# IrisRainbowNeko/HCP-Diffusion

Hardware: AMD Instinct MI355X
Metric: training images/sec (whole node), SD1.5 LoRA 512px bs=4/GPU (higher is better)
Workload: dtype bf16; 1 GPU; SD1.5 UNet LoRA rank=8 bf16, bs=4/GPU, 512x512 (64x64 latents), 77-token context, random-init weights, cached latents, grad-ckpt off; global_batch=4, parallelism=dp1, rccl_ranks=1, comm=none, hip_graph=True, gradient_checkpointing=False

## Files before the change

### hcp_diffusion_amd/csrc/attention.hip

```cpp
#include "attn_dma.h"

namespace {
using namespace hcp_attn;

HCP_KERNEL(256) attn_dkv_convert_kernel(AttnParams p, int B, int C) {
    const int cv = C / 4;
    const long total = (long)B * p.Nk * cv;
    const size_t slab = (size_t)B * p.Nk * C;
    for (long i = (long)blockIdx.x * blockDim.x + threadIdx.x; i < total; i += (long)gridDim.x * blockDim.x) {
        const int c = (int)(i % cv) * 4; long r = i / cv; const int n = (int)(r % p.Nk); const int b = (int)(r / p.Nk);
        const size_t e = ((size_t)b * p.Nk + n) * C + c;
        hcp_f32x4 k4 = *(const hcp_f32x4*)(p.dk32 + e);
        hcp_f32x4 v4 = *(const hcp_f32x4*)(p.dv32 + e);
        for (int s = 1; s < p.qsplit; ++s) {
            const hcp_f32x4 ks = *(const hcp_f32x4*)(p.dk32 + s * slab + e); k4 += ks;
            const hcp_f32x4 vs = *(const hcp_f32x4*)(p.dv32 + s * slab + e); v4 += vs;
        }
        hcp_bf16x4 wk, wv;
#pragma unroll
        for (int q = 0; q < 4; ++q) { wk[q] = (short)hcp_f2bf(k4[q]); wv[q] = (short)hcp_f2bf(v4[q]); }
        *(hcp_bf16x4*)(p.dK + (size_t)b * p.k_bs + (size_t)n * p.k_rs + c) = wk;
        *(hcp_bf16x4*)(p.dV + (size_t)b * p.v_bs + (size_t)n * p.v_rs + c) = wv;
    }
}

constexpr int kMinQTilesPerSplit = 16, kSplitTargetWgs = 256;
HCP_TUNABLE(int, g_attn_cfg, -1);

constexpr int VAR_FWD = VAR_PRODUCT | VAR_LSUM;
constexpr int VAR_PRE_BASE = VAR_XCD | VAR_ONES | VAR_PRE;
constexpr int VAR_FWD_PRE = VAR_PRE_BASE | VAR_LSUM;
template <int D, int QT, int NW>
int launch_fwd(AttnParams& p, int B, hipStream_t stream) {
    const int n = hcp_cdiv(p.Nq, 16 * QT * NW) * p.H * B;
    if (p.kbias || p.causal) HCP_LAUNCH((attn2_fwd_kernel<D, QT, true, VAR_PRODUCT, NW>), dim3(n), dim3(64 * NW), fwd_smem<D>(), stream, p);
    else if (p.pre) HCP_LAUNCH((attn2_fwd_kernel<D, QT, false, VAR_FWD_PRE, NW>), dim3(n), dim3(64 * NW), fwd_smem<D>(), stream, p);
    else HCP_LAUNCH((attn2_fwd_kernel<D, QT, false, VAR_FWD, NW>), dim3(n), dim3(64 * NW), fwd_smem<D>(), stream, p);
    HCP_LAUNCH_CHECK("attn_fwd");
}
template <int D, int QT>
int launch_dq(AttnParams& p, int B, hipStream_t stream) {
    const int n = hcp_cdiv(p.Nq, 64 * QT) * p.H * B;
    if (p.kbias || p.causal) HCP_LAUNCH((attn2_bwd_dq_kernel<D, QT, true, VAR_PRODUCT>), dim3(n), dim3(256), fwd_smem<D>(), stream, p);
    else if (p.pre) HCP_LAUNCH((attn2_bwd_dq_kernel<D, QT, false, VAR_PRE_BASE>), dim3(n), dim3(256), fwd_smem<D>(), stream, p);
    else HCP_LAUNCH((attn2_bwd_dq_kernel<D, QT, false, VAR_PRODUCT>), dim3(n), dim3(256), fwd_smem<D>(), stream, p);
    HCP_LAUNCH_CHECK("attn_bwd_dq");
}
template <int D, int KT>
void plan_dkv(AttnParams& p, int B, float* ws, size_t ws_bytes) {
    const int nkv = hcp_cdiv(p.Nk, 64 * KT);
    const int nqt = hcp_cdiv(p.Nq, KVT);
    int qsplit = 1;
    const long base = (long)nkv * p.H * B;
    const size_t need1 = (size_t)2 * B * p.Nk * p.H * D * sizeof(float);
    if (base < 256 && nqt >= 8 && ws && ws_bytes >= 2 * need1) {
        const bool ovr = g_attn_cfg >= 0 && (g_attn_cfg >> 8);
        const int min_tiles = ovr ? ((g_attn_cfg >> 8) & 255) : kMinQTilesPerSplit;
        const int target = ovr ? 256 * ((g_attn_cfg >> 16) & 15) : kSplitTargetWgs;
        qsplit = (int)((target + base - 1) / base);
        if (qsplit > nqt / min_tiles) qsplit = nqt / min_tiles;
        if ((size_t)qsplit > ws_bytes / need1) qsplit = (int)(ws_bytes / need1);
        if (qsplit < 2) qsplit = 1;
    }
    p.qsplit = qsplit;
    if (qsplit > 1) { p.dk32 = ws; p.dv32 = ws + (size_t)qsplit * B * p.Nk * p.H * D; }
}
template <int D, int KT>
int launch_dkv(AttnParams& p, int B, hipStream_t stream) {
    const int nkv = hcp_cdiv(p.Nk, 64 * KT);
    const int qsplit = p.qsplit;
    const int n = nkv * qsplit * p.H * B;
    if (p.kbias || p.causal) HCP_LAUNCH((attn2_bwd_dkv_kernel<D, KT, true, VAR_PRODUCT>), dim3(n), dim3(256), dkv_smem<D>(), stream, p);
    else if (p.pre) HCP_LAUNCH((attn2_bwd_dkv_kernel<D, KT, false, VAR_PRE_BASE>), dim3(n), dim3(256), dkv_smem<D>(), stream, p);
    else HCP_LAUNCH((attn2_bwd_dkv_kernel<D, KT, false, VAR_PRODUCT>), dim3(n), dim3(256), dkv_smem<D>(), stream, p);
    if (qsplit > 1) {
        long tot = (long)B * p.Nk * (p.H * D / 4);
        int g = (int)((tot + 255) / 256); if (g > 2048) g = 2048;
        HCP_LAUNCH(attn_dkv_convert_kernel, dim3(g), dim3(256), 0, stream, p, B, p.H * D);
    }
    HCP_LAUNCH_CHECK("attn_bwd_dkv");
}

template <int D> constexpr bool kWide = D <= 64;

template <int D>
int run_fwd(AttnParams& p, int B, hipStream_t stream) {
    const long bh = (long)B * p.H;
    bool wide = kWide<D> && bh * hcp_cdiv(p.Nq, 128) >= 512;
    bool w8 = (D == 40 || D == 80) && bh * hcp_cdiv(p.Nq, D == 40 ? 256 : 128) >= 256;
    if (g_attn_cfg >= 0 && !(g_attn_cfg & 16)) { wide = kWide<D> && (g_attn_cfg & 1); w8 = (D == 40 || D == 80) && (g_attn_cfg & 8); }
    if constexpr (D == 40) {
        if (w8) return wide ? launch_fwd<D, 2, 8>(p, B, stream) : launch_fwd<D, 1, 8>(p, B, stream);
        return wide ? launch_fwd<D, 2, 4>(p, B, stream) : launch_fwd<D, 1, 4>(p, B, stream);
    } else if constexpr (D == 80) {
        return w8 ? launch_fwd<D, 1, 8>(p, B, stream) : launch_fwd<D, 1, 4>(p, B, stream);
    } else if constexpr (kWide<D>) {
        return wide ? launch_fwd<D, 2, 4>(p, B, stream) : launch_fwd<D, 1, 4>(p, B, stream);
    } else {
        return launch_fwd<D, 1, 4>(p, B, stream);
    }
}
template <int D>
int run_bwd(AttnParams& p, int B, float* ws, size_t ws_bytes, hipStream_t stream) {
    bool wq = kWide<D> && (long)B * p.H * hcp_cdiv(p.Nq, 128) >= 512, wk = kWide<D> && (long)B * p.H * hcp_cdiv(p.Nk, 128) >= 512;
    if (g_attn_cfg >= 0 && !(g_attn_cfg & 16)) { wq = kWide<D> && (g_attn_cfg & 2); wk = kWide<D> && (g_attn_cfg & 4); }
    if constexpr (kWide<D>) { if (wk) plan_dkv<D, 2>(p, B, ws, ws_bytes); else plan_dkv<D, 1>(p, B, ws, ws_bytes); }
    else plan_dkv<D, 1>(p, B, ws, ws_bytes);
    int e;
    if constexpr (kWide<D>) { e = wq ? launch_dq<D, 2>(p, B, stream) : launch_dq<D, 1>(p, B, stream); }
    else e = launch_dq<D, 1>(p, B, stream);
    if (e) return e;
    if constexpr (kWide<D>) { return wk ? launch_dkv<D, 2>(p, B, stream) : launch_dkv<D, 1>(p, B, stream); }
    return launch_dkv<D, 1>(p, B, stream);
}

int attn_check(const AttnParams& p, int B, int D) {
    HCP_REQUIRE(B > 0 && p.H > 0 && p.Nq > 0 && p.Nk > 0, "attention: empty problem");
    HCP_REQUIRE(D == 40 || D == 64 || D == 80 || D == 160, "attention: head_dim %d unsupported (40/64/80/160)", D);
    HCP_REQUIRE(p.q_rs % 8 == 0 && p.k_rs % 8 == 0 && p.v_rs % 8 == 0 && p.o_rs % 8 == 0, "attention: row strides must be multiples of 8");
    HCP_REQUIRE(p.q_bs % 8 == 0 && p.k_bs % 8 == 0 && p.v_bs % 8 == 0 && p.o_bs % 8 == 0, "attention: batch strides must be multiples of 8");
    return 0;
}

}

#if defined(HCP_TOOLS)
HCP_API int hcp_debug_set_attention_config(int cfg) { g_attn_cfg = cfg; return 0; }
#endif

HCP_API int hcp_attention_fwd(const void* Q, const void* K, const void* V, void* O, float* lse, int B, int H, int Nq, int Nk,
                              int D, long q_bs, int q_rs, long k_bs, int k_rs, long v_bs, int v_rs, long o_bs, int o_rs,
                              float scale, const float* key_bias, long key_bias_bs, int causal, hipStream_t stream) {
    AttnParams p = {};
    p.kbias = key_bias; p.kb_bs = key_bias_bs; p.causal = causal & 1; p.pre = (causal >> 1) & 1; p.B = B;
    p.Q = (const hcp_bf16*)Q; p.K = (const hcp_bf16*)K; p.V = (const hcp_bf16*)V; p.Out = (hcp_bf16*)O; p.lse = lse;
    p.q_bs = q_bs; p.q_rs = q_rs; p.k_bs = k_bs; p.k_rs = k_rs; p.v_bs = v_bs; p.v_rs = v_rs; p.o_bs = o_bs; p.o_rs = o_rs;
    p.H = H; p.Nq = Nq; p.Nk = Nk; p.scale = scale; p.qsplit = 1;
    HCP_REQUIRE(Q && K && V && O && lse, "hcp_attention_fwd: null pointer");
    HCP_REQUIRE(!(causal & 1) || Nq == Nk, "hcp_attention_fwd: causal masking is defined for self-attention (Nq == Nk)");
    HCP_REQUIRE(!(causal & ~3), "hcp_attention_fwd: unknown flag bits (1 = causal, 2 = Q pre-scaled)");
    HCP_REQUIRE(!p.pre || !(key_bias || p.causal), "hcp_attention_fwd: pre-scaled Q is provided for the unmasked kernels only");
    if (int e = attn_check(p, B, D)) return e;
    switch (D) {
        case 40: return run_fwd<40>(p, B, stream);
        case 64: return run_fwd<64>(p, B, stream);
        case 80: return run_fwd<80>(p, B, stream);
        default: return run_fwd<160>(p, B, stream);
    }
}

HCP_API int hcp_attention_bwd(const void* Q, const void* K, const void* V, const void* O, const void* dO, const float* lse,
                              float* delta, void* dQ, void* dK, void* dV, int B, int H, int Nq, int Nk, int D, long q_bs,
                              int q_rs, long k_bs, int k_rs, long v_bs, int v_rs, long o_bs, int o_rs, float scale,
                              const float* key_bias, long key_bias_bs, int causal, void* workspace, size_t workspace_bytes,
                              hipStream_t stream) {
    AttnParams p = {};
    p.kbias = key_bias; p.kb_bs = key_bias_bs; p.causal = causal & 1; p.pre = (causal >> 1) & 1; p.B = B;
    p.Q = (const hcp_bf16*)Q; p.K = (const hcp_bf16*)K; p.V = (const hcp_bf16*)V; p.O = (const hcp_bf16*)O;
    p.dO = (const hcp_bf16*)dO; p.lse = (float*)lse; p.delta = delta;
    p.dQ = (hcp_bf16*)dQ; p.dK = (hcp_bf16*)dK; p.dV = (hcp_bf16*)dV;
    p.q_bs = q_bs; p.q_rs = q_rs; p.k_bs = k_bs; p.k_rs = k_rs; p.v_bs = v_bs; p.v_rs = v_rs; p.o_bs = o_bs; p.o_rs = o_rs;
    p.H = H; p.Nq = Nq; p.Nk = Nk; p.scale = scale; p.qsplit = 1;
    HCP_REQUIRE(Q && K && V && O && dO && lse && delta && dQ && dK && dV, "hcp_attention_bwd: null pointer");
    HCP_REQUIRE(!(causal & 1) || Nq == Nk, "hcp_attention_bwd: causal masking is defined for self-attention (Nq == Nk)");
    HCP_REQUIRE(!(causal & ~3), "hcp_attention_bwd: unknown flag bits (1 = causal, 2 = Q pre-scaled)");
    HCP_REQUIRE(!p.pre || !(key_bias || p.causal), "hcp_attention_bwd: pre-scaled Q is provided for the unmasked kernels only");
    if (int e = attn_check(p, B, D)) return e;
    float* ws = (float*)workspace; const size_t wb = workspace ? workspace_bytes : 0;
    switch (D) {
        case 40: return run_bwd<40>(p, B, ws, wb, stream);
        case 64: return run_bwd<64>(p, B, ws, wb, stream);
        case 80: return run_bwd<80>(p, B, ws, wb, stream);
        default: return run_bwd<160>(p, B, ws, wb, stream);
    }
}
```

Baseline: 211.4 images/sec.

## Add fused short-key attention backward kernel for cross-attention

Adds a specialised backward kernel for attention with few keys (up to 128, or 80 for head_dim 160), as in SD cross-attention with 77 text tokens. Each block keeps all of K and V resident in LDS and loops over query tiles, computing dQ, dK and dV in a single pass instead of separate dQ and dKV kernels. The query dimension is split across blocks to fill the CUs, and the fp32 dK/dV partials are reduced in the existing convert kernel. The cost is large LDS use per block and a partial-sum workspace, and the path falls back to the old kernels when the workspace is too small.

```diff
diff --git a/hcp_diffusion_amd/csrc/attention.hip b/hcp_diffusion_amd/csrc/attention.hip
--- a/hcp_diffusion_amd/csrc/attention.hip
+++ b/hcp_diffusion_amd/csrc/attention.hip
@@ -1,4 +1,5 @@
 #include "attn_dma.h"
+#include "attn_short_key.h"
 
 namespace {
 using namespace hcp_attn;
@@ -81,6 +82,48 @@
     HCP_LAUNCH_CHECK("attn_bwd_dkv");
 }
 
+constexpr int kSkCUs = 256, kSkMinTiles = 1;
+template <int D, int NKB>
+bool plan_sk(AttnParams& p, int B, float* ws, size_t ws_bytes) {
+    if (p.causal || p.Nk > sk_max_keys<D>()) return false;
+    int forced = 0;
+    if (g_attn_cfg >= 0) {
+        if (!(g_attn_cfg & 32)) return false;
+        forced = (g_attn_cfg >> 20) & 255;
+    }
+    const long bh = (long)B * p.H;
+    const int nqt = hcp_cdiv(p.Nq, KVT);
+    int s = forced;
+    if (!s) {
+        s = (int)(kSkCUs * SkGeom<D, NKB>::WAVES / bh);
+        if (s > nqt / kSkMinTiles) s = nqt / kSkMinTiles;
+        if (s < 1) s = 1;
+    }
+    if (s > nqt) s = nqt;
+    s = hcp_cdiv(nqt, hcp_cdiv(nqt, s));
+    if (s > 1) {
+        const size_t one = (size_t)B * p.Nk * p.H * D;
+        if (!ws || ws_bytes / (2 * one * sizeof(float)) < (size_t)s) return false;
+        p.dk32 = ws; p.dv32 = ws + (size_t)s * one;
+    }
+    p.qsplit = s;
+    return true;
+}
+template <int D, int NKB>
+int launch_sk(AttnParams& p, int B, hipStream_t stream) {
+    constexpr size_t smem = SkGeom<D, NKB>::SMEM;
+    const int n = p.qsplit * p.H * B;
+    if (p.kbias) HCP_LAUNCH((attn_sk_bwd_kernel<D, NKB, true, VAR_PRODUCT>), dim3(n), dim3(256), smem, stream, p);
+    else if (p.pre) HCP_LAUNCH((attn_sk_bwd_kernel<D, NKB, false, VAR_PRE_BASE>), dim3(n), dim3(256), smem, stream, p);
+    else HCP_LAUNCH((attn_sk_bwd_kernel<D, NKB, false, VAR_PRODUCT>), dim3(n), dim3(256), smem, stream, p);
+    if (p.qsplit > 1) {
+        long tot = (long)B * p.Nk * (p.H * D / 4);
+        int g = (int)((tot + 255) / 256); if (g > 2048) g = 2048;
+        HCP_LAUNCH(attn_dkv_convert_kernel, dim3(g), dim3(256), 0, stream, p, B, p.H * D);
+    }
+    HCP_LAUNCH_CHECK("attn_bwd_short_key");
+}
+
 template <int D> constexpr bool kWide = D <= 64;
 
 template <int D>
@@ -102,6 +145,10 @@
 }
 template <int D>
 int run_bwd(AttnParams& p, int B, float* ws, size_t ws_bytes, hipStream_t stream) {
+    if constexpr (sk_max_keys<D>() > 80) {
+        if (p.Nk > 80 && plan_sk<D, 8>(p, B, ws, ws_bytes)) return launch_sk<D, 8>(p, B, stream);
+    }
+    if (p.Nk <= 80 && plan_sk<D, 5>(p, B, ws, ws_bytes)) return launch_sk<D, 5>(p, B, stream);
     bool wq = kWide<D> && (long)B * p.H * hcp_cdiv(p.Nq, 128) >= 512, wk = kWide<D> && (long)B * p.H * hcp_cdiv(p.Nk, 128) >= 512;
     if (g_attn_cfg >= 0 && !(g_attn_cfg & 16)) { wq = kWide<D> && (g_attn_cfg & 2); wk = kWide<D> && (g_attn_cfg & 4); }
     if constexpr (kWide<D>) { if (wk) plan_dkv<D, 2>(p, B, ws, ws_bytes); else plan_dkv<D, 1>(p, B, ws, ws_bytes); }
diff --git a/hcp_diffusion_amd/csrc/attn_short_key.h b/hcp_diffusion_amd/csrc/attn_short_key.h
--- /dev/null
+++ b/hcp_diffusion_amd/csrc/attn_short_key.h
@@ -0,0 +1,231 @@
+#pragma once
+#include "attn_dma.h"
+
+namespace hcp_attn {
+
+template <int D, int NKB> struct SkGeom {
+    using G = Geom<D>;
+    static constexpr int NKBE = (NKB + 1) & ~1;
+    static constexpr int NCH = NKBE / 2;
+    static constexpr int NKP = 16 * NKBE;
+    static constexpr int RSP = NKP + 8;
+    static constexpr int NT = NKB * G::NDV;
+    static constexpr int TPW = (NT + 3) / 4;
+    static constexpr size_t KV_BYTES = (size_t)2 * NKP * G::RS * 2;
+    static constexpr size_t QG_BYTES = (size_t)2 * G::IMG * 2;
+    static constexpr size_t PS_BYTES = (size_t)2 * KVT * RSP * 2;
+    static constexpr size_t BIAS_BYTES = (size_t)NKP * 4;
+    static constexpr size_t LDS_CU = 160 * 1024;
+    static constexpr int NBUF = KV_BYTES + 2 * QG_BYTES + PS_BYTES + BIAS_BYTES <= LDS_CU ? 2 : 1;
+    static constexpr size_t SMEM = KV_BYTES + NBUF * QG_BYTES + PS_BYTES + BIAS_BYTES;
+    static constexpr int WAVES = LDS_CU / SMEM >= 2 ? 2 : 1;
+};
+template <int D> constexpr int sk_max_keys() { return D == 160 ? 80 : 128; }
+
+template <int D, int NKB, bool KB, int VAR>
+HCP_WAVES_PER_SIMD((SkGeom<D, NKB>::WAVES)) HCP_KERNEL(256) attn_sk_bwd_kernel(AttnParams p) {
+    using G = Geom<D>;
+    using SG = SkGeom<D, NKB>;
+    constexpr bool PRE = (VAR & VAR_PRE) != 0;
+    constexpr bool RAW = (VAR & VAR_RAW) != 0 && !PRE;
+    static_assert(PRE || RAW, "short-key backward: raw-unit or pre-scaled scores");
+    HCP_DYN_SMEM(smem);
+    hcp_bf16* sK = (hcp_bf16*)smem;
+    hcp_bf16* sV = sK + SG::NKP * G::RS;
+    hcp_bf16* sQG = sV + SG::NKP * G::RS;
+    hcp_bf16* sP = sQG + SG::NBUF * 2 * G::IMG;
+    hcp_bf16* sS = sP + KVT * SG::RSP;
+    float* sB = (float*)(sS + KVT * SG::RSP);
+    const int tid = threadIdx.x, lane = tid & 63, wave = hcp_uniform(tid >> 6);
+    const int fr = lane & 15, fg = lane >> 4;
+    const int S = p.qsplit;
+    int item = blockIdx.x;
+    if (VAR & VAR_XCD) item = xcd_work_item(item, gridDim.x);
+    const int bh = item / S, qs = item - bh * S, h = bh % p.H, b = bh / p.H;
+    const int nqt = (p.Nq + KVT - 1) / KVT;
+    const int per = (nqt + S - 1) / S;
+    const int it0 = qs * per, it1 = it0 + per < nqt ? it0 + per : nqt;
+    const hcp_bf16* Qb = p.Q + (size_t)b * p.q_bs + h * D;
+    const hcp_bf16* Kb = p.K + (size_t)b * p.k_bs + h * D;
+    const hcp_bf16* Vb = p.V + (size_t)b * p.v_bs + h * D;
+    const hcp_bf16* dOb = p.dO + (size_t)b * p.o_bs + h * D;
+    const hcp_bf16* Ob = p.O + (size_t)b * p.o_bs + h * D;
+    const float* lse_b = p.lse + ((size_t)b * p.H + h) * p.Nq;
+    const float cs = RAW ? p.scale * LOG2E : 1.0f;
+
+    for (int i = tid * 8; i < SG::NBUF * 2 * G::IMG; i += 256 * 8) *(hcp_bf16x8*)(sQG + i) = hcp_zero8();
+    for (int i = tid; i < SG::NKP * G::RG; i += 256) {
+        const int row = i / G::RG, g = i - row * G::RG;
+        const bool ok = row < p.Nk && g < G::REALG;
+        *(hcp_bf16x8*)(sK + row * G::RS + g * 8) = ok ? *(const hcp_bf16x8*)(Kb + (size_t)row * p.k_rs + g * 8) : hcp_zero8();
+        *(hcp_bf16x8*)(sV + row * G::RS + g * 8) = ok ? *(const hcp_bf16x8*)(Vb + (size_t)row * p.v_rs + g * 8) : hcp_zero8();
+    }
+    if (KB)
+        for (int i = tid; i < SG::NKP; i += 256)
+            sB[i] = (i < p.Nk && p.kbias) ? p.kbias[(size_t)b * p.kb_bs + i] * (RAW ? 1.0f / p.scale : LOG2E) : 0.f;
+    TileDma<D> dma;
+    dma.init(wave, lane, p.q_rs, p.o_rs);
+    auto nvalid_q = [&](int q0) { const int n = p.Nq - q0; return n < KVT ? n : KVT; };
+    auto fetch = [&](int it, hcp_bf16* dst) {
+        dma.issue(Qb + (size_t)it * KVT * p.q_rs, p.q_rs, dOb + (size_t)it * KVT * p.o_rs, p.o_rs, nvalid_q(it * KVT), dst, wave);
+    };
+    const int qrow = wave * 16 + fr;
+    hcp_bf16x8 of[G::NQK];
+    float lv = 0.f;
+#pragma unroll
+    for (int s = 0; s < G::NQK; ++s) of[s] = hcp_zero8();
+    auto load_o = [&](int it) {
+        const int row = it * KVT + qrow;
+#pragma unroll
+        for (int s = 0; s < G::NQK; ++s) {
+            const int dc = s * 32 + fg * 8;
+            of[s] = (row < p.Nq && dc < D) ? *(const hcp_bf16x8*)(Ob + (size_t)row * p.o_rs + dc) : hcp_zero8();
+        }
+        lv = row < p.Nq ? lse_b[row] : 0.f;
+    };
+    HCP_SYNC();
+    if (it0 < it1) { load_o(it0); fetch(it0, sQG); }
+    hcp_dma_wait_all();
+    HCP_SYNC();
+
+    hcp_f32x4 dk[SG::TPW], dv[SG::TPW];
+#pragma unroll
+    for (int j = 0; j < SG::TPW; ++j) { hcp_f32x4 z = {0.f, 0.f, 0.f, 0.f}; dk[j] = z; dv[j] = z; }
+    const int kfull = fr * G::RS + fg * 8;
+    const int ktail = fr * G::RS + ((G::NFULL * 32 + fg * 8) < D ? G::NFULL * 32 + fg * 8 : D);
+    const int tfrag = (4 * fg + (fr >> 2)) * G::RS + 4 * (fr & 3);
+    const int pfrag = (4 * fg + (fr >> 2)) * SG::RSP + 4 * (fr & 3);
+    hcp_bf16x4 dqw[G::NDV];
+    int dq_row = p.Nq;
+    auto flush_dq = [&]() {
+        if (dq_row < p.Nq) {
+            hcp_bf16* orow = p.dQ + (size_t)b * p.q_bs + (size_t)dq_row * p.q_rs + h * D;
+#pragma unroll
+            for (int d = 0; d < G::NDV; ++d)
+                if (d * 16 + 4 * fg < D) *(hcp_bf16x4*)(orow + d * 16 + 4 * fg) = dqw[d];
+        }
+        dq_row = p.Nq;
+    };
+    for (int it = it0; it < it1; ++it) {
+        const int q0 = it * KVT;
+        const hcp_bf16* sQ = sQG + (SG::NBUF == 2 ? ((it - it0) & 1) : 0) * 2 * G::IMG;
+        const hcp_bf16* sG = sQ + G::IMG;
+        float dpart = 0.f;
+#pragma unroll
+        for (int s = 0; s < G::NQK; ++s) {
+            const hcp_bf16x8 g = *(const hcp_bf16x8*)(sG + wave * 16 * G::RS + (s < G::NFULL ? kfull + s * 32 : ktail));
+#pragma unroll
+            for (int e = 0; e < 8; ++e) dpart += hcp_bf2f((unsigned short)of[s][e]) * hcp_bf2f((unsigned short)g[e]);
+        }
+        dpart += hcp_shfl_xor(dpart, 16); dpart += hcp_shfl_xor(dpart, 32);
+        const float l2 = q0 + qrow < p.Nq ? lv * LOG2E / cs : 0.f;
+        const hcp_f32x4 nl4 = {-l2, -l2, -l2, -l2}, nd4 = {-dpart, -dpart, -dpart, -dpart};
+        flush_dq();
+        if (it + 1 < it1) {
+            load_o(it + 1);
+            if (SG::NBUF == 2) fetch(it + 1, sQG + (((it + 1 - it0) & 1) * 2 * G::IMG));
+        }
+        hcp_f32x4 sc[SG::NKBE], dp[SG::NKBE];
+#pragma unroll
+        for (int s = 0; s < G::NQK; ++s) {
+            const int off = s < G::NFULL ? kfull + s * 32 : ktail;
+            const hcp_bf16x8 qa = *(const hcp_bf16x8*)(sQ + wave * 16 * G::RS + off);
+            const hcp_bf16x8 ga = *(const hcp_bf16x8*)(sG + wave * 16 * G::RS + off);
+#pragma unroll
+            for (int kb = 0; kb < NKB; ++kb) {
+                const hcp_bf16x8 kf = *(const hcp_bf16x8*)(sK + kb * 16 * G::RS + off);
+                const hcp_bf16x8 vf = *(const hcp_bf16x8*)(sV + kb * 16 * G::RS + off);
+                hcp_f32x4 init = nl4;
+                if (s == 0) {
+#pragma unroll
+                    for (int r = 0; r < 4; ++r) if (kb * 16 + 4 * fg + r >= p.Nk) init[r] = -INFINITY;
+                }
+                sc[kb] = hcp_mfma16(kf, qa, s == 0 ? init : sc[kb]);
+                dp[kb] = hcp_mfma16(vf, ga, s == 0 ? nd4 : dp[kb]);
+            }
+        }
+        hcp_bf16x8 df[SG::NCH];
+#pragma unroll
+        for (int kb = 0; kb < SG::NKBE; ++kb) {
+            hcp_bf16x4 pw, sw;
+#pragma unroll
+            for (int r = 0; r < 4; ++r) {
+                float pr = 0.f, ds = 0.f;
+                if (kb < NKB) {
+                    pr = hcp_exp2((KB ? sc[kb][r] + sB[kb * 16 + 4 * fg + r] : sc[kb][r]) * cs);
+                    ds = pr * dp[kb][r];
+                }
+                pw[r] = (short)hcp_f2bf(pr); sw[r] = (short)hcp_f2bf(ds);
+                df[kb / 2][(kb & 1) * 4 + r] = sw[r];
+            }
+            if (kb < NKB) {
+                *(hcp_bf16x4*)(sP + qrow * SG::RSP + kb * 16 + 4 * fg) = pw;
+                *(hcp_bf16x4*)(sS + qrow * SG::RSP + kb * 16 + 4 * fg) = sw;
+            }
+        }
+        hcp_f32x4 dq[G::NDV];
+#pragma unroll
+        for (int d = 0; d < G::NDV; ++d) {
+            hcp_f32x4 acc = {0.f, 0.f, 0.f, 0.f};
+#pragma unroll
+            for (int c = 0; c < SG::NCH; ++c) {
+                const hcp_bf16* a = sK + tfrag + (2 * c) * 16 * G::RS + d * 16;
+                acc = hcp_mfma16(join8(hcp_lds_read_tr4(a), hcp_lds_read_tr4(a + 16 * G::RS)), df[c], acc);
+            }
+            dq[d] = acc;
+        }
+#pragma unroll
+        for (int d = 0; d < G::NDV; ++d)
+#pragma unroll
+            for (int r = 0; r < 4; ++r) dqw[d][r] = (short)hcp_f2bf(dq[d][r] * (PRE ? LN2 : p.scale));
+        dq_row = q0 + qrow;
+        HCP_SYNC();
+#pragma unroll
+        for (int j = 0; j < SG::TPW; ++j) {
+            const int i = wave + 4 * j;
+            if (i < SG::NT) {
+                const int kb = i / G::NDV, d = i - kb * G::NDV;
+#pragma unroll
+                for (int s2 = 0; s2 < 2; ++s2) {
+                    const int off = tfrag + (2 * s2) * 16 * G::RS + d * 16;
+                    const int poff = pfrag + (2 * s2) * 16 * SG::RSP + kb * 16;
+                    const hcp_bf16x8 qa = join8(hcp_lds_read_tr4(sQ + off), hcp_lds_read_tr4(sQ + off + 16 * G::RS));
+                    const hcp_bf16x8 ga = join8(hcp_lds_read_tr4(sG + off), hcp_lds_read_tr4(sG + off + 16 * G::RS));
+                    const hcp_bf16x8 pf = join8(hcp_lds_read_tr4(sP + poff), hcp_lds_read_tr4(sP + poff + 16 * SG::RSP));
+                    const hcp_bf16x8 sf = join8(hcp_lds_read_tr4(sS + poff), hcp_lds_read_tr4(sS + poff + 16 * SG::RSP));
+                    dv[j] = hcp_mfma16(ga, pf, dv[j]);
+                    dk[j] = hcp_mfma16(qa, sf, dk[j]);
+                }
+            }
+        }
+        if (SG::NBUF == 1 && it + 1 < it1) {
+            HCP_SYNC();
+            fetch(it + 1, sQG);
+        }
+        hcp_dma_wait_all();
+        HCP_SYNC();
+    }
+    flush_dq();
+    const float kscale = PRE ? LN2 : p.scale;
+#pragma unroll
+    for (int j = 0; j < SG::TPW; ++j) {
+        const int i = wave + 4 * j;
+        if (i >= SG::NT) continue;
+        const int kb = i / G::NDV, d = i - kb * G::NDV;
+        const int key = kb * 16 + fr, col = d * 16 + 4 * fg;
+        if (key >= p.Nk || col >= D) continue;
+        if (S > 1) {
+            const size_t e = (size_t)qs * p.B * p.Nk * (p.H * D) + ((size_t)b * p.Nk + key) * (p.H * D) + h * D + col;
+            *(hcp_f32x4*)(p.dk32 + e) = dk[j] * kscale;
+            *(hcp_f32x4*)(p.dv32 + e) = dv[j];
+        } else {
+            hcp_bf16x4 wk, wv;
+#pragma unroll
+            for (int r = 0; r < 4; ++r) { wk[r] = (short)hcp_f2bf(dk[j][r] * kscale); wv[r] = (short)hcp_f2bf(dv[j][r]); }
+            *(hcp_bf16x4*)(p.dK + (size_t)b * p.k_bs + (size_t)key * p.k_rs + h * D + col) = wk;
+            *(hcp_bf16x4*)(p.dV + (size_t)b * p.v_bs + (size_t)key * p.v_rs + h * D + col) = wv;
+        }
+    }
+}
+
+}
```

Result: no change. 212.8 images/sec, median of 6 (+0.6%).
